# xxh0523/Py_PSNODE

Hardware: AMD Instinct MI355X
Metric: integrated state-steps/sec (batch x steps/s), RK4 neural-ODE, batch 4096 (higher is better)
Workload: dtype f32; 1 GPU; ode01 rk4: B=4096 trajectories/GPU x 1000 steps, x8 z2 H64, fp32, h=0.01, no events; kernel=mfma_wave, trajectories_total=4096, world_size_seen=1, device_count=1, collective=none, outputs_finite=True

## Files before the change

py_psnode_amd/csrc/psnode_mfma_x.h:

```cpp
#pragma once
#include <type_traits>

#include "psnode_launch.h"
#include "psnode_pack.h"

namespace psnode {
namespace {

typedef float f4 __attribute__((ext_vector_type(4)));
typedef float f2 __attribute__((ext_vector_type(2)));

__host__ __device__ constexpr int l1_dim(int m) { return 4 * ((m & 3) >> 1) + 2 * ((m & 3) & 1) + (m >= 4 ? 1 : 0); }

__host__ __device__ constexpr int l4_k(int m, int lane) { return 32 * (m >> 2) + 4 * ((lane >> 2) & 7) + (m & 3); }
__host__ __device__ constexpr int l4_dim(int lane) { return 4 * (lane >> 5) + (lane & 3); }
__host__ __device__ constexpr int l4_bias_dim(int r, int lane) { return ((lane >> 2) & 7) == 0 ? 4 * (lane >> 5) + r : -1; }

template <int ABID>
__device__ __forceinline__ f4 mfx(float a, float b, f4 c) { return __builtin_amdgcn_mfma_f32_4x4x1f32(a, b, c, 4, ABID, 0); }
__device__ __forceinline__ f4 mfn(float a, float b, f4 c) { return __builtin_amdgcn_mfma_f32_4x4x1f32(a, b, c, 0, 0, 0); }
template <int BLGP>
__device__ __forceinline__ f4 mfl(float a, float b, f4 c) { return __builtin_amdgcn_mfma_f32_4x4x1f32(a, b, c, 0, 0, BLGP); }

__device__ __forceinline__ f4 quad_transpose(const f4 v) {
// ... 117 lines not shown
    accB = mfx<BB>(hA[1], wk[4 * BB + 1], accB);
    accA = mfx<BB>(hA[2], wk[4 * BB + 2], accA);
    accB = mfx<BB>(hA[3], wk[4 * BB + 3], accB);
}
template <bool SC>
__device__ __forceinline__ f4 elu_x(const f4 v) {
    if constexpr (SC) return elu_quad_scaled(v);
    else return elu_quad(v);
}
template <bool SC, int ORD>
__device__ __forceinline__ f4 hh_layer(const float (&wk)[64], const float bias, const f4 hA, XMask& m) {
    f4 accA = f4{bias, bias, bias, bias}, accB = f4{0.f, 0.f, 0.f, 0.f};
    hh_block<0>(wk, hA, accA, accB); hh_block<1>(wk, hA, accA, accB); hh_block<2>(wk, hA, accA, accB); hh_block<3>(wk, hA, accA, accB);
    hh_block<4>(wk, hA, accA, accB); hh_block<5>(wk, hA, accA, accB); hh_block<6>(wk, hA, accA, accB); hh_block<7>(wk, hA, accA, accB);
    hh_block<8>(wk, hA, accA, accB); hh_block<9>(wk, hA, accA, accB); hh_block<10>(wk, hA, accA, accB); hh_block<11>(wk, hA, accA, accB);
    hh_block<12>(wk, hA, accA, accB); hh_block<13>(wk, hA, accA, accB); hh_block<14>(wk, hA, accA, accB); hh_block<15>(wk, hA, accA, accB);
    return quad_transpose_seq<ORD>(elu_x<SC>(accA + accB), m);
}

template <int BB>
__device__ __forceinline__ void hh_block_acc(const float (&wk)[64], const f4 hA, f4& accA, f4& accB) {
    asm volatile(
        "v_mfma_f32_4x4x1_16b_f32 %0, %2, %6, %0 cbsz:4 abid:%10\n\t"
        "v_mfma_f32_4x4x1_16b_f32 %1, %3, %7, %1 cbsz:4 abid:%10\n\t"
        "s_nop 0\n\t"
        "v_mfma_f32_4x4x1_16b_f32 %0, %4, %8, %0 cbsz:4 abid:%10\n\t"
        "v_mfma_f32_4x4x1_16b_f32 %1, %5, %9, %1 cbsz:4 abid:%10\n\t"
        "s_nop 0"
        : "+v"(accA), "+v"(accB)
        : "v"(hA[0]), "v"(hA[1]), "v"(hA[2]), "v"(hA[3]), "a"(wk[4 * BB + 0]), "a"(wk[4 * BB + 1]), "a"(wk[4 * BB + 2]), "a"(wk[4 * BB + 3]), "n"(BB));
}
template <bool SC, int ORD>
__device__ __forceinline__ f4 hh_layer_acc(const float (&wk)[64], const float bias, const f4 hA, XMask& m) {
    f4 accA = f4{bias, bias, bias, bias}, accB = f4{0.f, 0.f, 0.f, 0.f};
    asm volatile("s_nop 1" : "+v"(accA), "+v"(accB));
    hh_block_acc<0>(wk, hA, accA, accB); hh_block_acc<1>(wk, hA, accA, accB); hh_block_acc<2>(wk, hA, accA, accB); hh_block_acc<3>(wk, hA, accA, accB);
    hh_block_acc<4>(wk, hA, accA, accB); hh_block_acc<5>(wk, hA, accA, accB); hh_block_acc<6>(wk, hA, accA, accB); hh_block_acc<7>(wk, hA, accA, accB);
    hh_block_acc<8>(wk, hA, accA, accB); hh_block_acc<9>(wk, hA, accA, accB); hh_block_acc<10>(wk, hA, accA, accB); hh_block_acc<11>(wk, hA, accA, accB);
    hh_block_acc<12>(wk, hA, accA, accB); hh_block_acc<13>(wk, hA, accA, accB); hh_block_acc<14>(wk, hA, accA, accB); hh_block_acc<15>(wk, hA, accA, accB);
    asm volatile("s_nop 3" : "+v"(accA), "+v"(accB));
    return quad_transpose_seq<ORD>(elu_x<SC>(accA + accB), m);
}

template <int Q0, int NQ>
__device__ __forceinline__ f4 ext_mfmas(const float (&we)[16], const float eA, f4 acc) {
    if constexpr (NQ > 0) {
        acc = mfx<Q0>(eA, we[Q0], acc);
        return ext_mfmas<Q0 + 1, NQ - 1>(we, eA, acc);
    } else {
        return acc;
    }
}

constexpr int kXWaves = 4;

inline bool span32_ok(const long long B, const long long sb, const long long cols) {
    if (sb < 0 || B < 1) return false;
    const unsigned long long last = (unsigned long long)(B - 1) * (unsigned long long)sb + (unsigned long long)cols;
    return last < (1ull << 30);
}

}
}
```

py_psnode_amd/csrc/psnode_mfma_x.hip:

```cpp
#include <string.h>

#include "psnode_mfma_x.h"

namespace psnode {
namespace {

struct XRegs {
    static constexpr int W2 = 0, W3 = 64, W1X = 128, W1E = 136, W1A = 152, B1 = 168, B2 = 169, B3 = 170, W4A = 171, B4C = 179, COUNT = 187;
};
struct PackX {
    int xd, zd, n, hreal;
    float sc;
    const float *w1, *b1, *w2, *b2, *w3, *b3, *w4, *b4;
    float* out;
};
__global__ void pack_x_kernel(const PackX p) {
    const int H = p.hreal, n = p.n, xd = p.xd, ne = p.zd, K1 = 3 * n;
    const float kLog2e = p.sc;
    for (int idx = blockIdx.x * blockDim.x + threadIdx.x; idx < XRegs::COUNT * 64; idx += gridDim.x * blockDim.x) {
        const int reg = idx >> 6, l = idx & 63, u = l;
        float v = 0.0f;
        if (reg < XRegs::W1X) {
            const int k = reg & 63;
            const float* W = reg < XRegs::W3 ? p.w2 : p.w3;
// ... 66 lines not shown
            } else {
                if (st01) stg<float>((gptr<float>)(uintptr_t)sx_run, xooff, xs[0]);
                if (st23) stg<float>((gptr<float>)(uintptr_t)sx_run, xooff + 4u, xs[1]);
            }
            if (sa_on) {
                stg<f4>((gptr<float>)(uintptr_t)sa_run, saoff, h0);
                stg<f4>((gptr<float>)(uintptr_t)(sa_run + sa_layer), saoff, h1);
                stg<f4>((gptr<float>)(uintptr_t)(sa_run + 2 * sa_layer), saoff, h2);
            }
            sx_run += xo_step;
            sa_run += 3 * sa_layer;
        }
    }
}

template <int METHOD, int NZM, bool SAVE, bool ROLES = false>
__global__ __launch_bounds__(64 * kXWaves * (ROLES ? 2 : 1)) void integrate_x_kernel(const IntegrateDev a, const float* __restrict__ pack) {
    static_assert(!ROLES || SAVE, "the two-role form is the saving forward's");
    extern __shared__ __attribute__((aligned(16))) float xring[];
    const int l = threadIdx.x & 63;
    const int wv = __builtin_amdgcn_readfirstlane(threadIdx.x >> 6);
    if constexpr (ROLES) {
        if (wv >= kXWaves) { x_store_role<METHOD>(a, xring, l, wv - kXWaves); return; }
    }
    const int b = l >> 2, c = l & 3, rho = l >> 4;
    const long long tile = (long long)blockIdx.x * kXWaves + wv;
    if (!ROLES && tile * 4 >= a.B) return;
    const bool valid = tile * 4 + c < a.B;
    const long long tr = valid ? tile * 4 + c : a.B - 1;
    const int xd = a.xd, zd = a.zd, ne = zd, n = xd + zd;
    const bool true_x = !SAVE && (a.flags & PSNODE_FLAG_INPUT_TRUE_X) != 0;

    const float* pw = pack + l;
    float w2[64], w3[64], w1x[8], w1e[16], w4a[8];
    f4 b4c;
#pragma unroll
    for (int k = 0; k < 64; ++k) { w2[k] = pw[(XRegs::W2 + k) * 64]; w3[k] = pw[(XRegs::W3 + k) * 64]; }
#pragma unroll
    for (int m = 0; m < 8; ++m) { w1x[m] = pw[(XRegs::W1X + m) * 64]; w4a[m] = pw[(XRegs::W4A + m) * 64]; }
#pragma unroll
    for (int q = 0; q < 16; ++q) w1e[q] = q < 4 * NZM ? pw[(XRegs::W1E + q) * 64] : 0.0f;
    const float b1 = pw[XRegs::B1 * 64], b2 = pw[XRegs::B2 * 64], b3 = pw[XRegs::B3 * 64];
#pragma unroll
    for (int r = 0; r < 4; ++r) b4c[r] = pw[(XRegs::B4C + r) * 64];

    const int d01 = 4 * (rho >> 1) + 2 * (rho & 1), d23 = d01 + 1;
    const float* a0p = a.a0 + tr * n;
    f4 c0 = f4{b1, b1, b1, b1};
    {
        const float a0A = b < n ? a0p[b] : 0.0f;
        float wa[16];
#pragma unroll
        for (int q = 0; q < 16; ++q) wa[q] = pw[(XRegs::W1A + q) * 64];
        c0 = ext_mfmas<0, 16>(wa, a0A, c0);
    }
    const int ecol = b < ne ? b : (b < 2 * ne ? b - ne : 0);
    const float a0e = b < ne ? a0p[xd + b] : 0.0f;
    const bool eon = b < 2 * ne;
    f2 X = f2{0.0f, 0.0f};
    {
        const float* x0 = a.x.p + tr * a.x.sb;
        if (d01 < xd) X[0] = x0[d01];
        if (d23 < xd) X[1] = x0[d23];
    }
    const bool storer = (b & 3) == 0 && valid;
    if (a.T < 2 && storer) {
        float* row = a.xo + tr * xd;
        if (d01 < xd) row[d01] = X[0];
        if (d23 < xd) row[d23] = X[1];
    }
    const int nT = (int)a.T;
    if (nT < 2) return;

    const long long tst = a.t.st, xst = a.x.st;
    const bool has_z = zd > 0, has_zj = has_z && a.zj != nullptr;
    const long long zst = has_z ? a.z.st : 0, zje = has_zj ? a.zje : 0;
    const unsigned toff = (unsigned)(tr * a.t.sb) * 4u;
    const unsigned zoff = has_z ? (unsigned)(tr * a.z.sb + ecol) * 4u : toff;
    const unsigned zjoff = has_zj ? (unsigned)(tr * a.zjb + ecol) * 4u : toff;
    const float* zbase = has_z ? a.z.p : a.t.p;
    const float* zjbase = has_zj ? a.zj : a.t.p;
    const int d01c = d01 < xd ? d01 : 0, d23c = d23 < xd ? d23 : 0;
    const unsigned xtoff01 = (unsigned)(tr * a.x.sb + d01c) * 4u, xtoff23 = (unsigned)(tr * a.x.sb + d23c) * 4u;
    const unsigned xooff = (unsigned)(tr * xd + d01) * 4u;
    bool fast_rt = !true_x && (xd & 1) == 0;
    if (fast_rt && a.ev) {
        int any = -1;
        for (int i = l; i + 1 < nT; i += 64) any = max(any, a.ev[i]);
        fast_rt = __builtin_amdgcn_ballot_w64(any >= 0) == 0;
    }
    const int hp = SAVE ? padded_hidden(a.de.out_dim[0]) : 0;
    constexpr int kStg = METHOD == PSNODE_EULER ? 1 : (METHOD == PSNODE_MIDPOINT ? 2 : 4);
    const size_t sa_layer = SAVE ? (PSNODE_K1X_SAVE_ABL >= 3 ? (size_t)256 : (size_t)a.B * hp) : 0;
    const size_t sa_stage = SAVE ? (PSNODE_K1X_SAVE_ABL == 4 ? (size_t)768 : 3 * (size_t)a.B * hp) : 0;
    float* sa_run = SAVE ? a.sact : nullptr;
    float* sx_run = SAVE ? a.sxst : nullptr;
    const unsigned saoff = !SAVE ? 0u : (PSNODE_K1X_SAVE_ABL == 3 ? (unsigned)(tile * 768 + c * 64 + 4 * b) * 4u
                                         : (PSNODE_K1X_SAVE_ABL == 4 ? (unsigned)(tile * 768 * kStg + c * 64 + 4 * b) * 4u
                                                                     : (unsigned)(tr * hp + 4 * b) * 4u));
    const bool sa_on = SAVE && valid && 4 * b < hp && PSNODE_K1X_SAVE_ABL != 1;
    float* ring_mine = ROLES ? xring + (size_t)wv * kXRingFloats : nullptr;
    int ring_sl = 0, ring_half = 0;
    auto time_loop = [&](auto fast_tag) {
    constexpr bool FAST = decltype(fast_tag)::value;
    auto as_g = [](const float* q) { return (gptr<const float>)(uintptr_t)q; };
    auto load_evb = [&](const int blk) -> int {
        const int i = blk * 64 + l;
        const int v = (a.ev && i + 1 < nT) ? a.ev[i] : -1;
        __builtin_amdgcn_s_waitcnt(0x0F70);
        return v;
    };
    int evb = FAST ? -1 : load_evb(0);
    int ev_cur = FAST ? -1 : __builtin_amdgcn_readlane(evb, 0);
    float t_cur = ldg<float>(as_g(a.t.p), toff), t_nxt = ldg<float>(as_g(a.t.p + tst), toff);
    float e_nxt = (!FAST && ev_cur >= 0) ? ldg<float>(as_g(zjbase + (long long)ev_cur * zje), zjoff) : ldg<float>(as_g(zbase), zoff);
    const float* trun = a.t.p + 2 * tst;
    const float* zrun = zbase + zst;
    float* xo_run = a.xo;
    const long long xo_step = a.B * xd;
    const float* xt_run = a.x.p;
    const bool st01 = storer && d01 < xd, st23 = storer && d23 < xd;
    const bool pair_ok = FAST || (xd & 1) == 0;
    auto store_row = [&](float* row) {
        if (pair_ok) {
            if (st01) stg<f2>((gptr<float>)(uintptr_t)row, xooff, X);
        } else {
            if (st01) stg<float>((gptr<float>)(uintptr_t)row, xooff, X[0]);
            if (st23) stg<float>((gptr<float>)(uintptr_t)row, xooff + 4u, X[1]);
        }
    };

    XMask vm = xmask_even();
    auto rhs = [&](auto par_tag, const f2 s, const f4 cz) -> f2 {
        const float s01 = s[0], s23 = s[1];
        constexpr int P = decltype(par_tag)::value;
        f4 accA = cz, accB = f4{0.f, 0.f, 0.f, 0.f};
        accA = mfx<0>(s01, w1x[0], accA);  accB = mfx<4>(s01, w1x[1], accB);
        accA = mfx<8>(s01, w1x[2], accA);  accB = mfx<12>(s01, w1x[3], accB);
        accA = mfx<0>(s23, w1x[4], accA);  accB = mfx<4>(s23, w1x[5], accB);
        accA = mfx<8>(s23, w1x[6], accA);  accB = mfx<12>(s23, w1x[7], accB);
        f4 hA = quad_transpose_seq<P>(elu_x<!SAVE>(accA + accB), vm);
        float* slot = ROLES ? ring_mine + (ring_half * 4 + ring_sl) * kXSlotFloats : nullptr;
        if constexpr (ROLES) {
            *reinterpret_cast<f2*>(slot + 768 + 2 * l) = s;
            *reinterpret_cast<f4*>(slot + 4 * l) = hA;
        } else if constexpr (SAVE) {
            if (pair_ok) {
                if (st01) stg<f2>((gptr<float>)(uintptr_t)sx_run, xooff, s);
            } else {
                if (st01) stg<float>((gptr<float>)(uintptr_t)sx_run, xooff, s01);
                if (st23) stg<float>((gptr<float>)(uintptr_t)sx_run, xooff + 4u, s23);
            }
            if constexpr (PSNODE_K1X_SAVE_ABL != 2) sx_run += xo_step;
            if (sa_on) stg<f4>((gptr<float>)(uintptr_t)sa_run, saoff, hA);
        }
        hA = hh_layer<!SAVE, 1 - P>(w2, b2, hA, vm);
        if constexpr (ROLES) *reinterpret_cast<f4*>(slot + 256 + 4 * l) = hA;
        else if constexpr (SAVE) { if (sa_on) stg<f4>((gptr<float>)(uintptr_t)(sa_run + sa_layer), saoff, hA); }
        hA = hh_layer<!SAVE, P>(w3, b3, hA, vm);
        if constexpr (ROLES) {
            *reinterpret_cast<f4*>(slot + 512 + 4 * l) = hA;
            if (++ring_sl == 4) { lds_barrier(); ring_sl = 0; ring_half ^= 1; }
        } else if constexpr (SAVE) {
            if (sa_on) stg<f4>((gptr<float>)(uintptr_t)(sa_run + 2 * sa_layer), saoff, hA);
            if constexpr (PSNODE_K1X_SAVE_ABL != 2) sa_run += sa_stage;
        }
        return l4_out(w4a, b4c, hA);
    };

    auto step = [&](const int k, float& tprev, float& tuse, float& euse, auto pf_tag, auto wait_tag, auto lag_tag) {
        constexpr bool PF = decltype(pf_tag)::value;
        constexpr int WAITN = decltype(wait_tag)::value;
        constexpr bool LAG = decltype(lag_tag)::value;
        constexpr int NSAVE = (SAVE && !ROLES) ? 4 * (METHOD == PSNODE_EULER ? 1 : (METHOD == PSNODE_MIDPOINT ? 2 : 4)) : 0;
        constexpr int RDEPTH = WAITN >= 100 ? WAITN - 100 : (WAITN == 4 ? 2 : 1);
        constexpr int WN = WAITN == 0 ? 0 : (1 + NSAVE) + (RDEPTH - 1) * (3 + NSAVE);
        static_assert(WN <= 63, "vmcnt is 6 bits");
        if (pair_ok && WN > 0) __builtin_amdgcn_s_waitcnt(0x0F70 | (WN & 15) | ((WN >> 4) << 14));
        else __builtin_amdgcn_s_waitcnt(0x0F70);
        const float h_ = tuse - tprev;
        if constexpr (!LAG) tprev = tuse;
        const float eA = eon ? (b < ne ? euse - a0e : euse) : 0.0f;
        f2 s = X;
        if constexpr (!FAST) {
            if (true_x) {
                const float v01 = ldg<float>(as_g(xt_run), xtoff01), v23 = ldg<float>(as_g(xt_run), xtoff23);
                __builtin_amdgcn_s_waitcnt(0x0F70);
                s = f2{d01 < xd ? v01 : 0.0f, d23 < xd ? v23 : 0.0f};
            }
            xt_run += xst;
        }
        if constexpr (PF) {
            if constexpr (LAG) tprev = ldg<float>(as_g(trun), toff);
            else tuse = ldg<float>(as_g(trun), toff);
            if constexpr (FAST) {
                euse = ldg<float>(as_g(zrun), zoff);
            } else {
                if (((k + 1) & 63) == 0) evb = load_evb((k + 1) >> 6);
                ev_cur = __builtin_amdgcn_readlane(evb, (k + 1) & 63);
                const bool jump = __builtin_amdgcn_readfirstlane(ev_cur) >= 0;
                const float* zr = jump ? zjbase + (long long)ev_cur * zje : zrun;
                euse = ldg<float>(as_g(zr), jump ? zjoff : zoff);
            }
            trun += tst;
            zrun += zst;
        }
        store_row(xo_run);
        xo_run += xo_step;
        const f4 cz = ext_mfmas<0, 4 * NZM>(w1e, eA, c0);
        using P0 = std::integral_constant<int, 0>;
        using P1 = std::integral_constant<int, 1>;
        if constexpr (METHOD == PSNODE_EULER) vm = xmask_even();
        const f2 k1 = rhs(P0{}, s, cz);
        if constexpr (METHOD == PSNODE_EULER) {
            X = s + h_ * k1;
        } else if constexpr (METHOD == PSNODE_MIDPOINT) {
            const float hh = 0.5f * h_;
            const f2 k2 = rhs(P1{}, s + k1 * hh, cz);
            X = s + h_ * k2;
        } else {
            const f2 k2 = rhs(P1{}, s + h_ * k1 * kOneThird, cz);
            const f2 k3 = rhs(P0{}, s + h_ * (k2 - k1 * kOneThird), cz);
            const f2 k4 = rhs(P1{}, s + h_ * (k1 - k2 + k3), cz);
            X = s + (k1 + 3.0f * (k2 + k3) + k4) * h_ * 0.125f;
        }
        if constexpr (SAVE && PSNODE_K1X_SAVE_ABL == 4) sa_run += 3 * (size_t)a.B * hp * kStg - (size_t)768 * kStg;
    };
    using W0 = std::integral_constant<int, 0>;
    using W1 = std::integral_constant<int, 1>;
    using W4 = std::integral_constant<int, 4>;
    using NOLAG = std::false_type;
    constexpr bool TWO_AHEAD = FAST && METHOD != PSNODE_RK4_38;
    constexpr bool TWO_SLOT = FAST && METHOD == PSNODE_RK4_38;
    constexpr int RING = (SAVE && !ROLES && FAST) ? (METHOD == PSNODE_RK4_38 ? 3 : (METHOD == PSNODE_MIDPOINT ? 4 : 4)) : 0;
    if constexpr (RING > 0) {
        using WR = std::integral_constant<int, 100 + RING>;
        float tq[RING], eq[RING];
        tq[0] = t_nxt; eq[0] = e_nxt;
#pragma unroll
        for (int j = 1; j < RING; ++j) {
            const int rt = j + 1 < nT ? j + 1 : nT - 1, rz = j < nT ? j : nT - 1;
            tq[j] = ldg<float>(as_g(a.t.p + (long long)rt * tst), toff);
            eq[j] = ldg<float>(as_g(zbase + (long long)rz * zst), zoff);
        }
        trun = a.t.p + (long long)(RING + 1) * tst;
        zrun = zbase + (long long)RING * zst;
        __builtin_amdgcn_s_waitcnt(0x0F70);
        int k = 0;
        for (; k + 2 * RING + 1 <= nT; k += RING) {
#pragma unroll
            for (int j = 0; j < RING; ++j) step(k + j, t_cur, tq[j], eq[j], std::true_type{}, WR{}, NOLAG{});
        }
        __builtin_amdgcn_s_waitcnt(0x0F70);
        int slot = 0;
        for (; k + 1 < nT; ++k) {
            const bool pf = k + RING + 2 <= nT;
#pragma unroll
            for (int j = 0; j < RING; ++j) {
                if (slot == j) {
                    if (pf) step(k, t_cur, tq[j], eq[j], std::true_type{}, W0{}, NOLAG{});
                    else step(k, t_cur, tq[j], eq[j], std::false_type{}, W0{}, NOLAG{});
                }
            }
            slot = slot + 1 == RING ? 0 : slot + 1;
        }
    } else if constexpr (TWO_AHEAD) {
        float t_n2 = ldg<float>(as_g(a.t.p + (nT > 2 ? 2 : 1) * tst), toff);
        float e_n2 = ldg<float>(as_g(zbase + zst), zoff);
        trun = a.t.p + 3 * tst;
        zrun = zbase + 2 * zst;
        __builtin_amdgcn_s_waitcnt(0x0F70);
        int k = 0;
        for (; k + 5 <= nT; k += 2) {
            step(k, t_cur, t_nxt, e_nxt, std::true_type{}, W4{}, NOLAG{});
            step(k + 1, t_cur, t_n2, e_n2, std::true_type{}, W4{}, NOLAG{});
        }
        if (k + 4 <= nT) {
            step(k, t_cur, t_nxt, e_nxt, std::true_type{}, W4{}, NOLAG{});
            ++k;
        }
        __builtin_amdgcn_s_waitcnt(0x0F70);
        for (; k + 1 < nT; ++k) {
            if (k & 1) step(k, t_cur, t_n2, e_n2, std::false_type{}, W0{}, NOLAG{});
            else step(k, t_cur, t_nxt, e_nxt, std::false_type{}, W0{}, NOLAG{});
        }
    } else if constexpr (TWO_SLOT) {
        using LAG = std::true_type;
        __builtin_amdgcn_s_waitcnt(0x0F70);
        int k = 0;
        for (; k + 4 <= nT; k += 2) {
            step(k, t_cur, t_nxt, e_nxt, std::true_type{}, W1{}, LAG{});
            step(k + 1, t_nxt, t_cur, e_nxt, std::true_type{}, W1{}, LAG{});
        }
        if (k + 3 <= nT) {
            step(k, t_cur, t_nxt, e_nxt, std::true_type{}, W1{}, LAG{});
            ++k;
        }
        if (k & 1) step(k, t_nxt, t_cur, e_nxt, std::false_type{}, W0{}, LAG{});
        else step(k, t_cur, t_nxt, e_nxt, std::false_type{}, W0{}, LAG{});
    } else {
        __builtin_amdgcn_s_waitcnt(0x0F70);
        for (int k = 0; k + 2 < nT; ++k) step(k, t_cur, t_nxt, e_nxt, std::true_type{}, W1{}, NOLAG{});
        step(nT - 2, t_cur, t_nxt, e_nxt, std::false_type{}, W0{}, NOLAG{});
    }
    store_row(xo_run);
    };
    if (fast_rt) time_loop(std::true_type{});
    else time_loop(std::false_type{});
    if constexpr (ROLES) { if (ring_sl != 0) lds_barrier(); }
}

#ifndef PSNODE_K1X_SAVE_ROLES
#define PSNODE_K1X_SAVE_ROLES 0
#endif
template <int METHOD, bool SAVE>
hipError_t launch_x_method(const IntegrateDev& a, const float* pack, hipStream_t s) {
    constexpr bool ROLES = SAVE && PSNODE_K1X_SAVE_ROLES;
    const long long tiles = (a.B + 3) / 4;
    const dim3 grid((unsigned)((tiles + kXWaves - 1) / kXWaves)), block(64 * kXWaves * (ROLES ? 2 : 1));
    const size_t lds = ROLES ? (size_t)kXWaves * kXRingFloats * sizeof(float) : 0;
    return pick<0, 1, 2, 3, 4>((2 * a.zd + 3) / 4, [&](auto nzm) {
// ... 42 lines not shown
```

py_psnode_amd/csrc/psnode_mfma_xd.hip:

```cpp
#include <string.h>

#include "psnode_mfma_x.h"

namespace psnode {
namespace {

__host__ __device__ constexpr int xd_drow(int rho) { return rho == 1 ? 2 : (rho == 2 ? 1 : rho); }
__host__ __device__ inline int xd_slot_of_block(int b, int nzv, int id) {
    const int ne = nzv + id, rho = b >> 2, j = b & 3, d = xd_drow(rho);
    const bool has = d < id;
    if (has && j < 2) return j == 0 ? nzv + d : ne + nzv + d;
    int idx = j - (has ? 2 : 0);
    for (int r = 0; r < rho; ++r) idx += 4 - (xd_drow(r) < id ? 2 : 0);
    if (idx >= 2 * nzv) return -1;
    return idx < nzv ? idx : ne + (idx - nzv);
}

struct XDRegs {
    static constexpr int W2 = 0, W3 = 64, W1X = 128, W1E = 136, W1A = 152, B1 = 168, B2 = 169, B3 = 170, W4A = 171, B4C = 179,
                         AW1X = 187, AW1E = 195, AW1A = 203, AB1 = 219, AB2 = 220, AB3 = 221, AW4A = 222, AB4C = 226, COUNT = 230;
    static constexpr int HH_F4 = 2 * 16 * 64;
};
struct PackXD {
    int xd, zd, vd, id, hreal;
// ... 122 lines not shown
        for (int q = 0; q < 16; ++q) wa[q] = pw[(XDRegs::W1A + q) * 64];
        c0 = ext_mfmas<0, 16>(wa, a0A, c0);
#pragma unroll
        for (int q = 0; q < 16; ++q) wa[q] = pw[(XDRegs::AW1A + q) * 64];
        c0a = ext_mfmas<0, 16>(wa, a0A, c0a);
    }
    const int q_de = xd_slot_of_block(b, nzv, idim);
    const int e_de = q_de < 0 ? -1 : (q_de < ne ? q_de : q_de - ne);
    const int kind_de = e_de < 0 ? 3 : (e_de < zd ? 0 : (e_de < nzv ? 1 : 2));
    const int col_de = kind_de == 0 ? e_de : (kind_de == 1 ? e_de - zd : 0);
    const bool sub_de = q_de >= 0 && q_de < ne;
    const float a0e = sub_de ? a0p[xd + q_de] : 0.0f;
    const int kind_ae = b < zd ? 0 : (b < nzv ? 1 : 3);
    const int col_ae = kind_ae == 0 ? b : (kind_ae == 1 ? b - zd : 0);
    float X01 = d01 < xd ? a.x_init[tr * xd + d01] : 0.0f, X23 = d23 < xd ? a.x_init[tr * xd + d23] : 0.0f;
    const bool storer = (b & 3) == 0 && valid;
    const bool st01 = storer && d01 < xd, st23 = storer && d23 < xd, sti = storer && xd_drow(rho) < idim;
    const bool pair_ok = (xd & 1) == 0;
    const unsigned xooff = (unsigned)(tr * xd + d01) * 4u, iooff = (unsigned)(tr * idim + xd_drow(rho)) * 4u;
    const int nT = (int)a.T;

    const long long tst = a.t.st;
    const bool has_z = zd > 0, has_v = vd > 0, has_zj = has_z && a.zj != nullptr, has_vj = has_v && a.vj != nullptr;
    const long long zst = has_z ? a.z.st : 0, vst = has_v ? a.v.st : 0, zje = has_zj ? a.zje : 0, vje = has_vj ? a.vje : 0;
    const unsigned toff = (unsigned)(tr * a.t.sb) * 4u;
    const float* zbase = has_z ? a.z.p : a.t.p;
    const float* vbase = has_v ? a.v.p : a.t.p;
    const float* zjbase = has_zj ? a.zj : a.t.p;
    const float* vjbase = has_vj ? a.vj : a.t.p;
    const bool de_v = kind_de == 1 || (kind_de >= 2 && !has_z && has_v), ae_v = kind_ae == 1 || (kind_ae >= 2 && !has_z && has_v);
    auto lane_off = [&](const bool isv, const int kind, const int col, const bool jump) -> unsigned {
        const int cc = kind <= 1 ? col : 0;
        const unsigned ov = (unsigned)(tr * (jump ? a.vjb : a.v.sb) + cc) * 4u, oz = (unsigned)(tr * (jump ? a.zjb : a.z.sb) + cc) * 4u;
        return isv ? ov : (has_z ? oz : toff);
    };
    const unsigned off_de = lane_off(de_v, kind_de, col_de, false), off_ae = lane_off(ae_v, kind_ae, col_ae, false);
    const unsigned joff_de = ((de_v && has_vj) || (!de_v && has_zj)) ? lane_off(de_v, kind_de, col_de, true) : toff;
    const unsigned joff_ae = ((ae_v && has_vj) || (!ae_v && has_zj)) ? lane_off(ae_v, kind_ae, col_ae, true) : toff;
    auto as_g = [](const float* q) { return (gptr<const float>)(uintptr_t)q; };
    auto row_val = [&](const float* zr, const float* vr, const bool isv, const unsigned off) -> float {
        const float* rp = isv ? vr : zr;
        return *(gptr<const float>)((gptr<const char>)(uintptr_t)rp + off);
    };

    const long long xo_step = a.B * xd, io_step = a.B * idim;
    const int hp = SAVE ? padded_hidden(a.de.out_dim[0]) : 0;
    const size_t sa_layer = SAVE ? (size_t)a.B * hp : 0, sae_layer = SAVE ? (size_t)a.T * a.B * hp : 0;
    float* sa_run = SAVE ? a.sact : nullptr;
    float* sx_run = SAVE ? a.sxst : nullptr;
    float* sae_run = SAVE ? a.saeact : nullptr;
    const unsigned saoff = SAVE ? (unsigned)(tr * hp + 4 * b) * 4u : 0u;
    const bool sa_on = SAVE && valid && 4 * b < hp;
    XMask vm = xmask_even();
    auto rhs = [&](auto par_tag, const float s01, const float s23, const f4 cz, float& k01, float& k23) {
        constexpr int P = decltype(par_tag)::value;
        f4 accA = cz, accB = f4{0.f, 0.f, 0.f, 0.f};
        accA = mfx<0>(s01, w1x[0], accA);  accB = mfx<4>(s01, w1x[1], accB);
        accA = mfx<8>(s01, w1x[2], accA);  accB = mfx<12>(s01, w1x[3], accB);
        accA = mfx<0>(s23, w1x[4], accA);  accB = mfx<4>(s23, w1x[5], accB);
        accA = mfx<8>(s23, w1x[6], accA);  accB = mfx<12>(s23, w1x[7], accB);
        f4 hA = quad_transpose_seq<P>(elu_x<!SAVE>(accA + accB), vm);
        if constexpr (SAVE) {
            if (pair_ok) {
                if (st01) stg<f2>((gptr<float>)(uintptr_t)sx_run, xooff, f2{s01, s23});
            } else {
                if (st01) stg<float>((gptr<float>)(uintptr_t)sx_run, xooff, s01);
                if (st23) stg<float>((gptr<float>)(uintptr_t)sx_run, xooff + 4u, s23);
            }
            sx_run += xo_step;
            if (sa_on) stg<f4>((gptr<float>)(uintptr_t)sa_run, saoff, hA);
        }
        hA = hh_layer<!SAVE, 1 - P>(w2, b2, hA, vm);
        if constexpr (SAVE) { if (sa_on) stg<f4>((gptr<float>)(uintptr_t)(sa_run + sa_layer), saoff, hA); }
        hA = hh_layer<!SAVE, P>(w3, b3, hA, vm);
        if constexpr (SAVE) {
            if (sa_on) stg<f4>((gptr<float>)(uintptr_t)(sa_run + 2 * sa_layer), saoff, hA);
            sa_run += 3 * sa_layer;
        }
        f4 p0 = b4c[0], p1 = b4c[1];
        p0 = mfn(w4a[0], hA[0], p0); p1 = mfn(w4a[4], hA[0], p1);
        p0 = mfn(w4a[1], hA[1], p0); p1 = mfn(w4a[5], hA[1], p1);
        p0 = mfn(w4a[2], hA[2], p0); p1 = mfn(w4a[6], hA[2], p1);
        p0 = mfn(w4a[3], hA[3], p0); p1 = mfn(w4a[7], hA[3], p1);
        const float q0 = fold32(p0[0], p1[0]), q1 = fold32(p0[1], p1[1]), q2 = fold32(p0[2], p1[2]), q3 = fold32(p0[3], p1[3]);
        k01 = fold16(q0, q2); k23 = fold16(q1, q3);
        row_sum2(k01, k23);
    };
    auto ae_eval = [&](const float s01, const float s23, const float eAE, float* rows = nullptr, const size_t lstride = 0) -> float {
        f4 accA = c0a, accB = f4{0.f, 0.f, 0.f, 0.f};
        accA = mfx<0>(s01, aw1x[0], accA);  accB = mfx<4>(s01, aw1x[1], accB);
        accA = mfx<8>(s01, aw1x[2], accA);  accB = mfx<12>(s01, aw1x[3], accB);
        accA = mfx<0>(s23, aw1x[4], accA);  accB = mfx<4>(s23, aw1x[5], accB);
        accA = mfx<8>(s23, aw1x[6], accA);  accB = mfx<12>(s23, aw1x[7], accB);
        accA = mfx<0>(eAE, aw1e[0], accA);  accB = mfx<1>(eAE, aw1e[1], accB);
        accA = mfx<2>(eAE, aw1e[2], accA);  accB = mfx<3>(eAE, aw1e[3], accB);
        accA = mfx<4>(eAE, aw1e[4], accA);  accB = mfx<5>(eAE, aw1e[5], accB);
        accA = mfx<6>(eAE, aw1e[6], accA);  accB = mfx<7>(eAE, aw1e[7], accB);
        XMask am = xmask_even();
        f4 hA = quad_transpose_seq<0>(elu_x<!SAVE>(accA + accB), am);
        if constexpr (SAVE) { if (sa_on) stg<f4>((gptr<float>)(uintptr_t)rows, saoff, hA); }
        hA = hh_layer_acc<!SAVE, 1>(aw2, ab2, hA, am);
        if constexpr (SAVE) { if (sa_on) stg<f4>((gptr<float>)(uintptr_t)(rows + lstride), saoff, hA); }
        hA = hh_layer_acc<!SAVE, 0>(aw3, ab3, hA, am);
        if constexpr (SAVE) { if (sa_on) stg<f4>((gptr<float>)(uintptr_t)(rows + 2 * lstride), saoff, hA); }
        f4 p0 = ab4c;
        p0 = mfn(aw4a[0], hA[0], p0);
        p0 = mfn(aw4a[1], hA[1], p0);
        p0 = mfn(aw4a[2], hA[2], p0);
        p0 = mfn(aw4a[3], hA[3], p0);
        float w = fold16(fold32(p0[0], p0[1]), fold32(p0[2], p0[3]));
        row_sum1(w);
        return w;
    };

    auto load_evb = [&](const int blk) -> int {
        const int i = blk * 64 + l;
        const int v = (a.ev && i + 1 < nT) ? a.ev[i] : -1;
        __builtin_amdgcn_s_waitcnt(0x0F70);
        return v;
    };
    auto store_rows = [&](float* xrow, float* irow, const float iw) {
        if (pair_ok) {
            if (st01) stg<f2>((gptr<float>)(uintptr_t)xrow, xooff, f2{X01, X23});
        } else {
            if (st01) stg<float>((gptr<float>)(uintptr_t)xrow, xooff, X01);
            if (st23) stg<float>((gptr<float>)(uintptr_t)xrow, xooff + 4u, X23);
        }
// ... 23 lines not shown
        constexpr bool TOP = decltype(top_tag)::value;
        if constexpr (SAVE) {
            constexpr int WN = 2 + 4 * kStg + (TOP ? 3 : 0);
            if (pair_ok) __builtin_amdgcn_s_waitcnt(0x0F70 | (WN & 15) | ((WN >> 4) << 14));
            else __builtin_amdgcn_s_waitcnt(0x0F70);
        } else {
            if (METHOD == PSNODE_RK4_38 && pair_ok) __builtin_amdgcn_s_waitcnt(0x0F72);
            else __builtin_amdgcn_s_waitcnt(0x0F70);
        }
    };
    __builtin_amdgcn_s_waitcnt(0x0F70);
    auto step = [&](const int k, auto last_tag) {
        constexpr bool LAST = decltype(last_tag)::value;
        wait_loads(std::true_type{});
        const float h_ = t_nxt - t_cur;
        t_cur = t_nxt;
        const int ev_now = ev_cur;
        const float i_k = icw;
        if (__builtin_amdgcn_readfirstlane(ev_now) >= 0) {
            const float ej = row_val(zjbase + (long long)ev_now * zje, vjbase + (long long)ev_now * vje, ae_v, joff_ae);
            __builtin_amdgcn_s_waitcnt(0x0F70);
            icw = ae_eval(X01, X23, kind_ae == 3 ? 0.0f : ej, SAVE ? a.sevact + (size_t)ev_now * 3 * sa_layer : nullptr, sa_layer);
            if constexpr (SAVE) {
                const int d = xd_drow(rho);
                if (storer && d < idim) {
                    float* er = a.sevi + ((size_t)ev_now * a.B + tr) * 16;
                    er[nzv + d] = icw;
                    er[ne + nzv + d] = icw;
                }
                __builtin_amdgcn_s_waitcnt(0x0F70);
            }
        }
        float eA = kind_de == 2 ? icw : e_de_nxt;
        eA = sub_de ? eA - a0e : eA;
        eA = kind_de == 3 ? 0.0f : eA;
        if constexpr (!LAST) {
            t_nxt = ldg<float>(as_g(trun), toff);
            trun += tst;
            if (((k + 1) & 63) == 0) evb = load_evb((k + 1) >> 6);
            ev_cur = __builtin_amdgcn_readlane(evb, (k + 1) & 63);
        }
        e_ae = row_val(zrun, vrun, ae_v, off_ae);
        if constexpr (!LAST) {
            if (__builtin_amdgcn_readfirstlane(ev_cur) >= 0)
                e_de_nxt = row_val(zjbase + (long long)ev_cur * zje, vjbase + (long long)ev_cur * vje, de_v, joff_de);
            else
                e_de_nxt = row_val(zrun, vrun, de_v, off_de);
        }
        zrun += zst;
        vrun += vst;
        store_rows(xo_run, io_run, i_k);
        xo_run += xo_step;
        io_run += io_step;
        const f4 cz = ext_mfmas<0, 16>(w1e, eA, c0);
        const float s01 = X01, s23 = X23;
        float k1a, k1b;
        using P0 = std::integral_constant<int, 0>;
        using P1 = std::integral_constant<int, 1>;
        vm = xmask_even();
        rhs(P0{}, s01, s23, cz, k1a, k1b);
        if constexpr (METHOD == PSNODE_EULER) {
            X01 = s01 + h_ * k1a; X23 = s23 + h_ * k1b;
        } else if constexpr (METHOD == PSNODE_MIDPOINT) {
            const float hh = 0.5f * h_;
            float k2a, k2b;
            rhs(P1{}, s01 + k1a * hh, s23 + k1b * hh, cz, k2a, k2b);
            X01 = s01 + h_ * k2a; X23 = s23 + h_ * k2b;
        } else {
            float k2a, k2b, k3a, k3b, k4a, k4b;
            rhs(P1{}, s01 + h_ * k1a * kOneThird, s23 + h_ * k1b * kOneThird, cz, k2a, k2b);
            rhs(P0{}, s01 + h_ * (k2a - k1a * kOneThird), s23 + h_ * (k2b - k1b * kOneThird), cz, k3a, k3b);
            rhs(P1{}, s01 + h_ * (k1a - k2a + k3a), s23 + h_ * (k1b - k2b + k3b), cz, k4a, k4b);
            X01 = s01 + (k1a + 3.0f * (k2a + k3a) + k4a) * h_ * 0.125f;
            X23 = s23 + (k1b + 3.0f * (k2b + k3b) + k4b) * h_ * 0.125f;
        }
        wait_loads(std::false_type{});
        icw = ae_eval(X01, X23, kind_ae == 3 ? 0.0f : e_ae, sae_run, sae_layer);
        if constexpr (SAVE) sae_run += sa_layer;
    };
#pragma unroll 1
    for (int k = 0; k + 2 < nT; ++k) step(k, std::false_type{});
    step(nT - 2, std::true_type{});
    store_rows(xo_run, io_run, icw);
}

}

bool mfma_x_dae_supported(const IntegrateDev& a) {
    const int nzv = a.zd + a.vd, ne = nzv + a.id, n = a.xd + ne;
    if (a.flags || a.xd < 1 || a.xd > 8 || a.zd < 0 || a.vd < 0 || a.id < 1 || a.id > 4 || nzv < 1 || ne > 8 || a.T >= (1ll << 31)) return false;
    const MlpDev &d = a.de, &g = a.ae;
    if (d.n_layers != 4 || g.n_layers != 4 || d.in_dim != 3 * n || d.out_dim[3] != a.xd || g.in_dim != n + a.xd + nzv || g.out_dim[3] != a.id) return false;
    const int h = d.out_dim[0];
    if (!(h >= 1 && h <= 64 && d.out_dim[1] == h && d.out_dim[2] == h && g.out_dim[0] == h && g.out_dim[1] == h && g.out_dim[2] == h)) return false;
    if (a.t.p && !span32_ok(a.B, a.t.sb, 1)) return false;
    if (a.zd > 0 && a.z.p && !span32_ok(a.B, a.z.sb, a.zd)) return false;
    if (a.vd > 0 && a.v.p && !span32_ok(a.B, a.v.sb, a.vd)) return false;
    if (a.zd > 0 && a.zj && !span32_ok(a.B, a.zjb, a.zd)) return false;
    if (a.vd > 0 && a.vj && !span32_ok(a.B, a.vjb, a.vd)) return false;
    if (a.sact) {
        if (!a.sxst || !a.saeact || (a.ev && (!a.sevact || !a.sevi))) return false;
        if (((uintptr_t)a.sact & 15) || ((uintptr_t)a.sxst & 7) || ((uintptr_t)a.saeact & 15) || ((uintptr_t)a.sevact & 15)) return false;
        if (!span32_ok(a.B, 64, 64)) return false;
    }
    return span32_ok(a.B, a.xd, a.xd) && span32_ok(a.B, a.id, a.id);
}
bool mfma_x_dae_preferred(const IntegrateDev& a) {
    if (a.kern == PSNODE_KERNEL_MFMA_TILE || a.kern == PSNODE_KERNEL_GENERIC || !mfma_x_dae_supported(a)) return false;
    if (a.sact) return a.kern == PSNODE_KERNEL_MFMA_WAVE;
    return a.kern == PSNODE_KERNEL_MFMA_WAVE || a.B <= 4608;
}
size_t mfma_xd_pack_floats() { return (size_t)XDRegs::COUNT * 64 + (size_t)XDRegs::HH_F4 * 4; }

hipError_t launch_mfma_xd(const IntegrateDev& a, float* pack, hipStream_t stream) {
    PackXD p;
    p.xd = a.xd; p.zd = a.zd; p.vd = a.vd; p.id = a.id; p.hreal = a.de.out_dim[0];
    set_layers(p, a.de);
    p.aw1 = a.ae.w[0]; p.ab1 = a.ae.bias[0]; p.aw2 = a.ae.w[1]; p.ab2 = a.ae.bias[1];
    p.aw3 = a.ae.w[2]; p.ab3 = a.ae.bias[2]; p.aw4 = a.ae.w[3]; p.ab4 = a.ae.bias[3];
    p.out = pack;
    p.sc = a.sact ? 1.0f : kLog2e;
    hipLaunchKernelGGL(pack_xd_kernel, dim3(32), dim3(256), 0, stream, p);
    hipError_t e = hipGetLastError();
    if (e != hipSuccess) return e;
    const long long tiles = (a.B + 3) / 4;
// ... 10 lines not shown
```

Measured before the change: 1.371 billion state-steps/s.

## Swap first-layer MFMA operand roles to drop per-stage quad transpose

Rewrites the first MLP layer with swapped A/B operands, using B-lane-group broadcast, so its output lands directly in the layout the hidden layers consume. This removes the quad_transpose that each RHS evaluation used to do after layer 1, and fixes the hidden-layer transpose parity instead of alternating it per stage. The transpose is moved onto the per-step constant bias term, which is computed once per step. Exogenous inputs now need one value per lane group, so each lane holds NE arrays of loads and offsets, which adds registers and extra loads per step.

Result: faster. 1.412 billion state-steps/s (median of 6 runs) (+3.0%).

```diff
diff --git a/py_psnode_amd/csrc/psnode_mfma_x.h b/py_psnode_amd/csrc/psnode_mfma_x.h
--- a/py_psnode_amd/csrc/psnode_mfma_x.h
+++ b/py_psnode_amd/csrc/psnode_mfma_x.h
@@ -193,6 +193,24 @@
     }
 }
 
+__device__ __forceinline__ f4 l1_swapped(const float (&w1x)[8], const f2 s, const f4 cz) {
+    f4 accA = cz, accB = f4{0.f, 0.f, 0.f, 0.f};
+    accA = mfl<4>(w1x[0], s[0], accA);  accB = mfl<5>(w1x[1], s[0], accB);
+    accA = mfl<6>(w1x[2], s[0], accA);  accB = mfl<7>(w1x[3], s[0], accB);
+    accA = mfl<4>(w1x[4], s[1], accA);  accB = mfl<5>(w1x[5], s[1], accB);
+    accA = mfl<6>(w1x[6], s[1], accA);  accB = mfl<7>(w1x[7], s[1], accB);
+    return accA + accB;
+}
+template <int Q0, int NQ, int NE>
+__device__ __forceinline__ f4 ext_mfmas_swapped(const float (&we)[16], const float (&eA)[NE], f4 acc) {
+    if constexpr (NQ > 0) {
+        acc = mfl<4 + (Q0 & 3)>(we[Q0], eA[Q0 >> 2], acc);
+        return ext_mfmas_swapped<Q0 + 1, NQ - 1, NE>(we, eA, acc);
+    } else {
+        return acc;
+    }
+}
+
 constexpr int kXWaves = 4;
 
 inline bool span32_ok(const long long B, const long long sb, const long long cols) {
diff --git a/py_psnode_amd/csrc/psnode_mfma_x.hip b/py_psnode_amd/csrc/psnode_mfma_x.hip
--- a/py_psnode_amd/csrc/psnode_mfma_x.hip
+++ b/py_psnode_amd/csrc/psnode_mfma_x.hip
@@ -142,11 +142,19 @@
         float wa[16];
 #pragma unroll
         for (int q = 0; q < 16; ++q) wa[q] = pw[(XRegs::W1A + q) * 64];
-        c0 = ext_mfmas<0, 16>(wa, a0A, c0);
-    }
-    const int ecol = b < ne ? b : (b < 2 * ne ? b - ne : 0);
-    const float a0e = b < ne ? a0p[xd + b] : 0.0f;
-    const bool eon = b < 2 * ne;
+        c0 = quad_transpose(ext_mfmas<0, 16>(wa, a0A, c0));
+    }
+    constexpr int NE = NZM > 0 ? NZM : 1;
+    int ecol[NE];
+    float a0e[NE];
+    bool eon[NE];
+#pragma unroll
+    for (int j = 0; j < NE; ++j) {
+        const int q = 4 * j + rho;
+        ecol[j] = q < ne ? q : (q < 2 * ne ? q - ne : 0);
+        a0e[j] = q < ne ? a0p[xd + q] : 0.0f;
+        eon[j] = q < 2 * ne;
+    }
     f2 X = f2{0.0f, 0.0f};
     {
         const float* x0 = a.x.p + tr * a.x.sb;
@@ -166,8 +174,12 @@
     const bool has_z = zd > 0, has_zj = has_z && a.zj != nullptr;
     const long long zst = has_z ? a.z.st : 0, zje = has_zj ? a.zje : 0;
     const unsigned toff = (unsigned)(tr * a.t.sb) * 4u;
-    const unsigned zoff = has_z ? (unsigned)(tr * a.z.sb + ecol) * 4u : toff;
-    const unsigned zjoff = has_zj ? (unsigned)(tr * a.zjb + ecol) * 4u : toff;
+    unsigned zoff[NE], zjoff[NE];
+#pragma unroll
+    for (int j = 0; j < NE; ++j) {
+        zoff[j] = has_z ? (unsigned)(tr * a.z.sb + ecol[j]) * 4u : toff;
+        zjoff[j] = has_zj ? (unsigned)(tr * a.zjb + ecol[j]) * 4u : toff;
+    }
     const float* zbase = has_z ? a.z.p : a.t.p;
     const float* zjbase = has_zj ? a.zj : a.t.p;
     const int d01c = d01 < xd ? d01 : 0, d23c = d23 < xd ? d23 : 0;
@@ -203,7 +215,10 @@
     int evb = FAST ? -1 : load_evb(0);
     int ev_cur = FAST ? -1 : __builtin_amdgcn_readlane(evb, 0);
     float t_cur = ldg<float>(as_g(a.t.p), toff), t_nxt = ldg<float>(as_g(a.t.p + tst), toff);
-    float e_nxt = (!FAST && ev_cur >= 0) ? ldg<float>(as_g(zjbase + (long long)ev_cur * zje), zjoff) : ldg<float>(as_g(zbase), zoff);
+    float e_nxt[NE];
+#pragma unroll
+    for (int j = 0; j < NE; ++j)
+        e_nxt[j] = (!FAST && ev_cur >= 0) ? ldg<float>(as_g(zjbase + (long long)ev_cur * zje), zjoff[j]) : ldg<float>(as_g(zbase), zoff[j]);
     const float* trun = a.t.p + 2 * tst;
     const float* zrun = zbase + zst;
     float* xo_run = a.xo;
@@ -221,15 +236,9 @@
     };
 
     XMask vm = xmask_even();
-    auto rhs = [&](auto par_tag, const f2 s, const f4 cz) -> f2 {
+    auto rhs = [&](const f2 s, const f4 cz) -> f2 {
         const float s01 = s[0], s23 = s[1];
-        constexpr int P = decltype(par_tag)::value;
-        f4 accA = cz, accB = f4{0.f, 0.f, 0.f, 0.f};
-        accA = mfx<0>(s01, w1x[0], accA);  accB = mfx<4>(s01, w1x[1], accB);
-        accA = mfx<8>(s01, w1x[2], accA);  accB = mfx<12>(s01, w1x[3], accB);
-        accA = mfx<0>(s23, w1x[4], accA);  accB = mfx<4>(s23, w1x[5], accB);
-        accA = mfx<8>(s23, w1x[6], accA);  accB = mfx<12>(s23, w1x[7], accB);
-        f4 hA = quad_transpose_seq<P>(elu_x<!SAVE>(accA + accB), vm);
+        f4 hA = elu_x<!SAVE>(l1_swapped(w1x, s, cz));
         float* slot = ROLES ? ring_mine + (ring_half * 4 + ring_sl) * kXSlotFloats : nullptr;
         if constexpr (ROLES) {
             *reinterpret_cast<f2*>(slot + 768 + 2 * l) = s;
@@ -244,10 +253,10 @@
             if constexpr (PSNODE_K1X_SAVE_ABL != 2) sx_run += xo_step;
             if (sa_on) stg<f4>((gptr<float>)(uintptr_t)sa_run, saoff, hA);
         }
-        hA = hh_layer<!SAVE, 1 - P>(w2, b2, hA, vm);
+        hA = hh_layer<!SAVE, 0>(w2, b2, hA, vm);
         if constexpr (ROLES) *reinterpret_cast<f4*>(slot + 256 + 4 * l) = hA;
         else if constexpr (SAVE) { if (sa_on) stg<f4>((gptr<float>)(uintptr_t)(sa_run + sa_layer), saoff, hA); }
-        hA = hh_layer<!SAVE, P>(w3, b3, hA, vm);
+        hA = hh_layer<!SAVE, 1>(w3, b3, hA, vm);
         if constexpr (ROLES) {
             *reinterpret_cast<f4*>(slot + 512 + 4 * l) = hA;
             if (++ring_sl == 4) { lds_barrier(); ring_sl = 0; ring_half ^= 1; }
@@ -258,19 +267,21 @@
         return l4_out(w4a, b4c, hA);
     };
 
-    auto step = [&](const int k, float& tprev, float& tuse, float& euse, auto pf_tag, auto wait_tag, auto lag_tag) {
+    auto step = [&](const int k, float& tprev, float& tuse, float (&euse)[NE], auto pf_tag, auto wait_tag, auto lag_tag) {
         constexpr bool PF = decltype(pf_tag)::value;
         constexpr int WAITN = decltype(wait_tag)::value;
         constexpr bool LAG = decltype(lag_tag)::value;
         constexpr int NSAVE = (SAVE && !ROLES) ? 4 * (METHOD == PSNODE_EULER ? 1 : (METHOD == PSNODE_MIDPOINT ? 2 : 4)) : 0;
         constexpr int RDEPTH = WAITN >= 100 ? WAITN - 100 : (WAITN == 4 ? 2 : 1);
-        constexpr int WN = WAITN == 0 ? 0 : (1 + NSAVE) + (RDEPTH - 1) * (3 + NSAVE);
+        constexpr int WN = WAITN == 0 ? 0 : (1 + NSAVE) + (RDEPTH - 1) * (2 + NE + NSAVE);
         static_assert(WN <= 63, "vmcnt is 6 bits");
         if (pair_ok && WN > 0) __builtin_amdgcn_s_waitcnt(0x0F70 | (WN & 15) | ((WN >> 4) << 14));
         else __builtin_amdgcn_s_waitcnt(0x0F70);
         const float h_ = tuse - tprev;
         if constexpr (!LAG) tprev = tuse;
-        const float eA = eon ? (b < ne ? euse - a0e : euse) : 0.0f;
+        float eA[NE];
+#pragma unroll
+        for (int j = 0; j < NE; ++j) eA[j] = eon[j] ? euse[j] - a0e[j] : 0.0f;
         f2 s = X;
         if constexpr (!FAST) {
             if (true_x) {
@@ -284,34 +295,36 @@
             if constexpr (LAG) tprev = ldg<float>(as_g(trun), toff);
             else tuse = ldg<float>(as_g(trun), toff);
             if constexpr (FAST) {
-                euse = ldg<float>(as_g(zrun), zoff);
+#pragma unroll
+                for (int j = 0; j < NE; ++j) euse[j] = ldg<float>(as_g(zrun), zoff[j]);
             } else {
                 if (((k + 1) & 63) == 0) evb = load_evb((k + 1) >> 6);
                 ev_cur = __builtin_amdgcn_readlane(evb, (k + 1) & 63);
                 const bool jump = __builtin_amdgcn_readfirstlane(ev_cur) >= 0;
                 const float* zr = jump ? zjbase + (long long)ev_cur * zje : zrun;
-                euse = ldg<float>(as_g(zr), jump ? zjoff : zoff);
+#pragma unroll
+                for (int j = 0; j < NE; ++j) {
+                    const unsigned zo = zoff[j], zjo = zjoff[j];
+                    euse[j] = ldg<float>(as_g(zr), jump ? zjo : zo);
+                }
             }
             trun += tst;
             zrun += zst;
         }
         store_row(xo_run);
         xo_run += xo_step;
-        const f4 cz = ext_mfmas<0, 4 * NZM>(w1e, eA, c0);
-        using P0 = std::integral_constant<int, 0>;
-        using P1 = std::integral_constant<int, 1>;
-        if constexpr (METHOD == PSNODE_EULER) vm = xmask_even();
-        const f2 k1 = rhs(P0{}, s, cz);
+        const f4 cz = ext_mfmas_swapped<0, 4 * NZM, NE>(w1e, eA, c0);
+        const f2 k1 = rhs(s, cz);
         if constexpr (METHOD == PSNODE_EULER) {
             X = s + h_ * k1;
         } else if constexpr (METHOD == PSNODE_MIDPOINT) {
             const float hh = 0.5f * h_;
-            const f2 k2 = rhs(P1{}, s + k1 * hh, cz);
+            const f2 k2 = rhs(s + k1 * hh, cz);
             X = s + h_ * k2;
         } else {
-            const f2 k2 = rhs(P1{}, s + h_ * k1 * kOneThird, cz);
-            const f2 k3 = rhs(P0{}, s + h_ * (k2 - k1 * kOneThird), cz);
-            const f2 k4 = rhs(P1{}, s + h_ * (k1 - k2 + k3), cz);
+            const f2 k2 = rhs(s + h_ * k1 * kOneThird, cz);
+            const f2 k3 = rhs(s + h_ * (k2 - k1 * kOneThird), cz);
+            const f2 k4 = rhs(s + h_ * (k1 - k2 + k3), cz);
             X = s + (k1 + 3.0f * (k2 + k3) + k4) * h_ * 0.125f;
         }
         if constexpr (SAVE && PSNODE_K1X_SAVE_ABL == 4) sa_run += 3 * (size_t)a.B * hp * kStg - (size_t)768 * kStg;
@@ -325,13 +338,16 @@
     constexpr int RING = (SAVE && !ROLES && FAST) ? (METHOD == PSNODE_RK4_38 ? 3 : (METHOD == PSNODE_MIDPOINT ? 4 : 4)) : 0;
     if constexpr (RING > 0) {
         using WR = std::integral_constant<int, 100 + RING>;
-        float tq[RING], eq[RING];
-        tq[0] = t_nxt; eq[0] = e_nxt;
+        float tq[RING], eq[RING][NE];
+        tq[0] = t_nxt;
+#pragma unroll
+        for (int i = 0; i < NE; ++i) eq[0][i] = e_nxt[i];
 #pragma unroll
         for (int j = 1; j < RING; ++j) {
             const int rt = j + 1 < nT ? j + 1 : nT - 1, rz = j < nT ? j : nT - 1;
             tq[j] = ldg<float>(as_g(a.t.p + (long long)rt * tst), toff);
-            eq[j] = ldg<float>(as_g(zbase + (long long)rz * zst), zoff);
+#pragma unroll
+            for (int i = 0; i < NE; ++i) eq[j][i] = ldg<float>(as_g(zbase + (long long)rz * zst), zoff[i]);
         }
         trun = a.t.p + (long long)(RING + 1) * tst;
         zrun = zbase + (long long)RING * zst;
@@ -356,7 +372,9 @@
         }
     } else if constexpr (TWO_AHEAD) {
         float t_n2 = ldg<float>(as_g(a.t.p + (nT > 2 ? 2 : 1) * tst), toff);
-        float e_n2 = ldg<float>(as_g(zbase + zst), zoff);
+        float e_n2[NE];
+#pragma unroll
+        for (int j = 0; j < NE; ++j) e_n2[j] = ldg<float>(as_g(zbase + zst), zoff[j]);
         trun = a.t.p + 3 * tst;
         zrun = zbase + 2 * zst;
         __builtin_amdgcn_s_waitcnt(0x0F70);
diff --git a/py_psnode_amd/csrc/psnode_mfma_xd.hip b/py_psnode_amd/csrc/psnode_mfma_xd.hip
--- a/py_psnode_amd/csrc/psnode_mfma_xd.hip
+++ b/py_psnode_amd/csrc/psnode_mfma_xd.hip
@@ -198,14 +198,8 @@
     const unsigned saoff = SAVE ? (unsigned)(tr * hp + 4 * b) * 4u : 0u;
     const bool sa_on = SAVE && valid && 4 * b < hp;
     XMask vm = xmask_even();
-    auto rhs = [&](auto par_tag, const float s01, const float s23, const f4 cz, float& k01, float& k23) {
-        constexpr int P = decltype(par_tag)::value;
-        f4 accA = cz, accB = f4{0.f, 0.f, 0.f, 0.f};
-        accA = mfx<0>(s01, w1x[0], accA);  accB = mfx<4>(s01, w1x[1], accB);
-        accA = mfx<8>(s01, w1x[2], accA);  accB = mfx<12>(s01, w1x[3], accB);
-        accA = mfx<0>(s23, w1x[4], accA);  accB = mfx<4>(s23, w1x[5], accB);
-        accA = mfx<8>(s23, w1x[6], accA);  accB = mfx<12>(s23, w1x[7], accB);
-        f4 hA = quad_transpose_seq<P>(elu_x<!SAVE>(accA + accB), vm);
+    auto rhs = [&](const float s01, const float s23, const f4 cz, float& k01, float& k23) {
+        f4 hA = elu_x<!SAVE>(l1_swapped(w1x, f2{s01, s23}, cz));
         if constexpr (SAVE) {
             if (pair_ok) {
                 if (st01) stg<f2>((gptr<float>)(uintptr_t)sx_run, xooff, f2{s01, s23});
@@ -216,9 +210,9 @@
             sx_run += xo_step;
             if (sa_on) stg<f4>((gptr<float>)(uintptr_t)sa_run, saoff, hA);
         }
-        hA = hh_layer<!SAVE, 1 - P>(w2, b2, hA, vm);
+        hA = hh_layer<!SAVE, 1>(w2, b2, hA, vm);
         if constexpr (SAVE) { if (sa_on) stg<f4>((gptr<float>)(uintptr_t)(sa_run + sa_layer), saoff, hA); }
-        hA = hh_layer<!SAVE, P>(w3, b3, hA, vm);
+        hA = hh_layer<!SAVE, 0>(w3, b3, hA, vm);
         if constexpr (SAVE) {
             if (sa_on) stg<f4>((gptr<float>)(uintptr_t)(sa_run + 2 * sa_layer), saoff, hA);
             sa_run += 3 * sa_layer;
@@ -348,25 +342,23 @@
         store_rows(xo_run, io_run, i_k);
         xo_run += xo_step;
         io_run += io_step;
-        const f4 cz = ext_mfmas<0, 16>(w1e, eA, c0);
+        vm = xmask_even();
+        const f4 cz = quad_transpose_seq<0>(ext_mfmas<0, 16>(w1e, eA, c0), vm);
         const float s01 = X01, s23 = X23;
         float k1a, k1b;
-        using P0 = std::integral_constant<int, 0>;
-        using P1 = std::integral_constant<int, 1>;
-        vm = xmask_even();
-        rhs(P0{}, s01, s23, cz, k1a, k1b);
+        rhs(s01, s23, cz, k1a, k1b);
         if constexpr (METHOD == PSNODE_EULER) {
             X01 = s01 + h_ * k1a; X23 = s23 + h_ * k1b;
         } else if constexpr (METHOD == PSNODE_MIDPOINT) {
             const float hh = 0.5f * h_;
             float k2a, k2b;
-            rhs(P1{}, s01 + k1a * hh, s23 + k1b * hh, cz, k2a, k2b);
+            rhs(s01 + k1a * hh, s23 + k1b * hh, cz, k2a, k2b);
             X01 = s01 + h_ * k2a; X23 = s23 + h_ * k2b;
         } else {
             float k2a, k2b, k3a, k3b, k4a, k4b;
-            rhs(P1{}, s01 + h_ * k1a * kOneThird, s23 + h_ * k1b * kOneThird, cz, k2a, k2b);
-            rhs(P0{}, s01 + h_ * (k2a - k1a * kOneThird), s23 + h_ * (k2b - k1b * kOneThird), cz, k3a, k3b);
-            rhs(P1{}, s01 + h_ * (k1a - k2a + k3a), s23 + h_ * (k1b - k2b + k3b), cz, k4a, k4b);
+            rhs(s01 + h_ * k1a * kOneThird, s23 + h_ * k1b * kOneThird, cz, k2a, k2b);
+            rhs(s01 + h_ * (k2a - k1a * kOneThird), s23 + h_ * (k2b - k1b * kOneThird), cz, k3a, k3b);
+            rhs(s01 + h_ * (k1a - k2a + k3a), s23 + h_ * (k1b - k2b + k3b), cz, k4a, k4b);
             X01 = s01 + (k1a + 3.0f * (k2a + k3a) + k4a) * h_ * 0.125f;
             X23 = s23 + (k1b + 3.0f * (k2b + k3b) + k4b) * h_ * 0.125f;
         }
```
